# SWivid/F5-TTS

Hardware: NVIDIA H100
Metric: mel_frames_per_sec (higher is better)
Workload: dtype fp16 operands / fp32 accumulate+state

## Files before the change

### f5_tts_b200/csrc/attn.cuh

```cuda
#pragma once
#include "common.cuh"
#include "kparams.h"
#include "wgmma.cuh"

namespace f5 {

__device__ __forceinline__ float ex2_approx(float x) {
  float y;
  asm("ex2.approx.ftz.f32 %0, %1;" : "=f"(y) : "f"(x));
  return y;
}

__global__ void __launch_bounds__(kAttnThreads, 1)
attn_fwd_wgmma_kernel(const __grid_constant__ CUtensorMap tmQKV, const AttnParams p) {
  extern __shared__ uint8_t smem_raw[];
  const uint32_t base = (smem_u32(smem_raw) + 1023u) & ~1023u;
  uint8_t* smem = smem_raw + (base - smem_u32(smem_raw));
  uint8_t* sQ = smem;
  uint8_t* sK = sQ + kAttnTile;
  uint8_t* sV = sK + kAttnStages * kAttnTile;
  uint64_t* bars = reinterpret_cast<uint64_t*>(sV + kAttnStages * kAttnTile);
  uint64_t* q_full = bars;
  uint64_t* k_full = q_full + 1;
  uint64_t* k_empty = k_full + kAttnStages;
  uint64_t* v_full = k_empty + kAttnStages;
  uint64_t* v_empty = v_full + kAttnStages;

  const int warp = threadIdx.x >> 5;
  const int qb = blockIdx.x, h = blockIdx.y, b = blockIdx.z;
  const int q0 = qb * kAttnBQ;
  const int col_q = h * 64, col_k = p.inner + h * 64, col_v = 2 * p.inner + h * 64;

  if (warp == 8 && elect_one()) {
    tma_prefetch_desc(&tmQKV);
    mbar_init(q_full, 1);
    for (int s = 0; s < kAttnStages; ++s) {
      mbar_init(&k_full[s], 1);
      mbar_init(&k_empty[s], 8);
      mbar_init(&v_full[s], 1);
      mbar_init(&v_empty[s], 8);
    }
    fence_mbar_init();
  }
  __syncthreads();
  pdl_wait();
  pdl_launch_dependents();
  const int kv_len = p.kv_len ? max(1, min(p.kv_len[b], p.seq)) : p.seq;
  const int n_kv = (kv_len + kAttnBKV - 1) / kAttnBKV;

  if (warp == 8) {
    if (elect_one()) {
      mbar_expect_tx(q_full, kAttnTile);
      tma_load_3d(sQ, &tmQKV, q_full, col_q, q0, b);
      for (int j = 0; j < n_kv; ++j) {
        const int s = j % kAttnStages;
        const uint32_t ph = (j / kAttnStages) & 1;
        mbar_wait(&k_empty[s], ph ^ 1);
        mbar_expect_tx(&k_full[s], kAttnTile);
        tma_load_3d(sK + s * kAttnTile, &tmQKV, &k_full[s], col_k, j * kAttnBKV, b);
        mbar_wait(&v_empty[s], ph ^ 1);
        mbar_expect_tx(&v_full[s], kAttnTile);
        tma_load_3d(sV + s * kAttnTile, &tmQKV, &v_full[s], col_v, j * kAttnBKV, b);
      }
    }
    return;
  }

  const int g = warp >> 2;
  const int lane = int(lane_id());
  const int r = 64 * g + 16 * (warp & 3) + (lane >> 2);
  const int c2 = 2 * (lane & 3);
  const uint64_t qdesc = make_wgmma_desc_sw128(smem_u32(sQ + g * (64 * 128)));
  float o[32];
#pragma unroll
  for (int i = 0; i < 32; ++i) o[i] = 0.0f;
  float m_run[2] = {-INFINITY, -INFINITY}, l_run[2] = {0.0f, 0.0f};
  mbar_wait(q_full, 0);
  for (int j = 0; j < n_kv; ++j) {
    const int s = j % kAttnStages;
    const uint32_t ph = (j / kAttnStages) & 1;
    const int kv_rem = kv_len - j * kAttnBKV;
    float sc[64];
    mbar_wait(&k_full[s], ph);
    const uint64_t kdesc = make_wgmma_desc_sw128(smem_u32(sK + s * kAttnTile));
    wgmma_fence();
#pragma unroll
    for (int k = 0; k < 4; ++k) wgmma_ss_n128(sc, qdesc + uint64_t(2 * k), kdesc + uint64_t(2 * k), k != 0);
    wgmma_commit();
    wgmma_wait<0>();
    wgmma_fence_regs(sc);
    __syncwarp();
    if (lane == 0) mbar_arrive(&k_empty[s]);
    if (kv_rem < kAttnBKV) {
#pragma unroll
      for (int i = 0; i < 64; ++i)
        if (8 * (i >> 2) + c2 + (i & 1) >= kv_rem) sc[i] = -INFINITY;
    }
    float alpha[2];
#pragma unroll
    for (int hr = 0; hr < 2; ++hr) {
      float mx = -INFINITY;
#pragma unroll
      for (int jj = 0; jj < 16; ++jj) mx = fmaxf(mx, fmaxf(sc[4 * jj + 2 * hr], sc[4 * jj + 2 * hr + 1]));
      mx = fmaxf(mx, __shfl_xor_sync(0xffffffffu, mx, 1));
      mx = fmaxf(mx, __shfl_xor_sync(0xffffffffu, mx, 2));
      const float m_new = fmaxf(m_run[hr], mx * p.scale_log2);
      alpha[hr] = ex2_approx(m_run[hr] - m_new);
      m_run[hr] = m_new;
      float sum = 0.0f;
#pragma unroll
      for (int jj = 0; jj < 16; ++jj) {
        const float e0 = ex2_approx(fmaf(sc[4 * jj + 2 * hr], p.scale_log2, -m_new));
        const float e1 = ex2_approx(fmaf(sc[4 * jj + 2 * hr + 1], p.scale_log2, -m_new));
        sc[4 * jj + 2 * hr] = e0;
        sc[4 * jj + 2 * hr + 1] = e1;
        sum += e0 + e1;
      }
      l_run[hr] = l_run[hr] * alpha[hr] + sum;
    }
#pragma unroll
    for (int jj = 0; jj < 8; ++jj) {
      o[4 * jj + 0] *= alpha[0];
      o[4 * jj + 1] *= alpha[0];
      o[4 * jj + 2] *= alpha[1];
      o[4 * jj + 3] *= alpha[1];
    }
    uint32_t pa[8][4];
#pragma unroll
    for (int kk = 0; kk < 8; ++kk) {
      pa[kk][0] = pack_half2(sc[8 * kk + 0], sc[8 * kk + 1]);
      pa[kk][1] = pack_half2(sc[8 * kk + 2], sc[8 * kk + 3]);
      pa[kk][2] = pack_half2(sc[8 * kk + 4], sc[8 * kk + 5]);
      pa[kk][3] = pack_half2(sc[8 * kk + 6], sc[8 * kk + 7]);
    }
    mbar_wait(&v_full[s], ph);
    wgmma_fence();
#pragma unroll
    for (int kk = 0; kk < 8; ++kk)
      wgmma_rs_n64_bt(o, pa[kk], make_wgmma_desc_sw128(smem_u32(sV + s * kAttnTile + kk * 16 * 128)), 1);
    wgmma_commit();
    wgmma_wait<0>();
    wgmma_fence_regs(o);
    __syncwarp();
    if (lane == 0) mbar_arrive(&v_empty[s]);
  }
#pragma unroll
  for (int hr = 0; hr < 2; ++hr) {
    float l = l_run[hr];
    l += __shfl_xor_sync(0xffffffffu, l, 1);
    l += __shfl_xor_sync(0xffffffffu, l, 2);
    const float inv_l = 1.0f / l;
    const int qrow = q0 + r + 8 * hr;
    if (qrow < p.seq) {
      __half* out = p.out + ((long long)b * p.seq + qrow) * p.inner + h * 64 + c2;
#pragma unroll
      for (int jj = 0; jj < 8; ++jj)
        *reinterpret_cast<uint32_t*>(out + 8 * jj) = pack_half2(o[4 * jj + 2 * hr] * inv_l, o[4 * jj + 2 * hr + 1] * inv_l);
    }
  }
}

}
```

### f5_tts_b200/csrc/common.cuh

```cuda
#pragma once
#include <cuda.h>
#include <cuda_fp16.h>
#include <cuda_runtime.h>
#include <stdint.h>
#include <stdio.h>

#ifndef F5_SPIN_TIMEOUT_CYCLES
#define F5_SPIN_TIMEOUT_CYCLES (4000000000LL)
#endif

namespace f5 {

__device__ __forceinline__ uint32_t smem_u32(const void* p) {
  return static_cast<uint32_t>(__cvta_generic_to_shared(p));
}
__device__ __forceinline__ uint32_t lane_id() { return threadIdx.x & 31; }

__device__ __forceinline__ bool elect_one() {
  uint32_t pred = 0;
  asm volatile(
      "{\n\t.reg .pred P;\n\t.reg .b32 R;\n\telect.sync R|P, 0xffffffff;\n\tselp.b32 %0, 1, 0, P;\n\t}\n"
      : "=r"(pred));
  return pred != 0;
}

__device__ __forceinline__ void mbar_init(uint64_t* bar, uint32_t count) {
  asm volatile("mbarrier.init.shared::cta.b64 [%0], %1;" ::"r"(smem_u32(bar)), "r"(count) : "memory");
}
__device__ __forceinline__ void fence_mbar_init() { asm volatile("fence.mbarrier_init.release.cluster;" ::: "memory"); }
__device__ __forceinline__ void mbar_expect_tx(uint64_t* bar, uint32_t bytes) {
  asm volatile("mbarrier.arrive.expect_tx.shared::cta.b64 _, [%0], %1;" ::"r"(smem_u32(bar)), "r"(bytes) : "memory");
}
__device__ __forceinline__ void mbar_arrive(uint64_t* bar) {
  asm volatile("mbarrier.arrive.shared::cta.b64 _, [%0];" ::"r"(smem_u32(bar)) : "memory");
}
__device__ __forceinline__ bool mbar_try_wait(uint64_t* bar, uint32_t parity) {
  uint32_t ok;
  asm volatile(
      "{\n\t.reg .pred P;\n\tmbarrier.try_wait.parity.shared::cta.b64 P, [%1], %2;\n\tselp.b32 %0, 1, 0, P;\n\t}\n"
      : "=r"(ok)
      : "r"(smem_u32(bar)), "r"(parity)
      : "memory");
  return ok != 0;
}
__device__ __forceinline__ void mbar_wait(uint64_t* bar, uint32_t parity) {
  if (mbar_try_wait(bar, parity)) return;
  long long t0 = clock64();
  while (!mbar_try_wait(bar, parity)) {
    if (clock64() - t0 > F5_SPIN_TIMEOUT_CYCLES) __trap();
  }
}

__device__ __forceinline__ bool mbar_test(uint64_t* bar, uint32_t parity) {
  uint32_t ok;
  asm volatile(
      "{\n\t.reg .pred p;\n\tmbarrier.test_wait.parity.shared::cta.b64 p, [%1], %2;\n\tselp.u32 %0, 1, 0, p;\n\t}"
      : "=r"(ok)
      : "r"(smem_u32(bar)), "r"(parity)
      : "memory");
  return ok != 0;
}

__device__ __forceinline__ void fence_proxy_async_smem() { asm volatile("fence.proxy.async.shared::cta;" ::: "memory"); }
__device__ __forceinline__ void fence_proxy_async_all() { asm volatile("fence.proxy.async;" ::: "memory"); }

__device__ __forceinline__ void tma_prefetch_desc(const CUtensorMap* m) {
  asm volatile("prefetch.tensormap [%0];" ::"l"(reinterpret_cast<uint64_t>(m)) : "memory");
}
__device__ __forceinline__ void tma_load_2d(void* smem_dst, const CUtensorMap* m, uint64_t* bar, int c0, int c1) {
  asm volatile(
      "cp.async.bulk.tensor.2d.shared::cluster.global.mbarrier::complete_tx::bytes [%0], [%1, {%3, %4}], [%2];" ::"r"(
          smem_u32(smem_dst)),
      "l"(reinterpret_cast<uint64_t>(m)), "r"(smem_u32(bar)), "r"(c0), "r"(c1)
      : "memory");
}
__device__ __forceinline__ void tma_load_3d(void* smem_dst, const CUtensorMap* m, uint64_t* bar, int c0, int c1,
                                            int c2) {
  asm volatile(
      "cp.async.bulk.tensor.3d.shared::cluster.global.mbarrier::complete_tx::bytes [%0], [%1, {%3, %4, %5}], [%2];" ::
          "r"(smem_u32(smem_dst)),
      "l"(reinterpret_cast<uint64_t>(m)), "r"(smem_u32(bar)), "r"(c0), "r"(c1), "r"(c2)
      : "memory");
}

__device__ __forceinline__ void tma_store_3d(const CUtensorMap* m, const void* smem_src, int c0, int c1, int c2) {
  asm volatile("cp.async.bulk.tensor.3d.global.shared::cta.bulk_group [%0, {%2, %3, %4}], [%1];" ::"l"(
                   reinterpret_cast<uint64_t>(m)),
               "r"(smem_u32(smem_src)), "r"(c0), "r"(c1), "r"(c2)
               : "memory");
}
__device__ __forceinline__ void tma_reduce_add_3d(const CUtensorMap* m, const void* smem_src, int c0, int c1, int c2) {
  asm volatile("cp.reduce.async.bulk.tensor.3d.global.shared::cta.add.tile.bulk_group [%0, {%2, %3, %4}], [%1];" ::"l"(
                   reinterpret_cast<uint64_t>(m)),
               "r"(smem_u32(smem_src)), "r"(c0), "r"(c1), "r"(c2)
               : "memory");
}
__device__ __forceinline__ void tma_store_commit() { asm volatile("cp.async.bulk.commit_group;" ::: "memory"); }
template <int N>
__device__ __forceinline__ void tma_store_wait_read() {
  asm volatile("cp.async.bulk.wait_group.read %0;" ::"n"(N) : "memory");
}
__device__ __forceinline__ void tma_store_wait_all() { asm volatile("cp.async.bulk.wait_group 0;" ::: "memory"); }
__device__ __forceinline__ void named_bar_sync(int id, int nthreads) {
  asm volatile("bar.sync %0, %1;" ::"r"(id), "r"(nthreads) : "memory");
}

__device__ __forceinline__ void tma_load_2d_multicast(void* smem_dst, const CUtensorMap* m, uint64_t* bar, int c0, int c1,
                                                      uint16_t cta_mask) {
  asm volatile(
      "cp.async.bulk.tensor.2d.shared::cluster.global.mbarrier::complete_tx::bytes.multicast::cluster [%0], [%1, {%3, "
      "%4}], [%2], %5;" ::"r"(smem_u32(smem_dst)),
      "l"(reinterpret_cast<uint64_t>(m)), "r"(smem_u32(bar)), "r"(c0), "r"(c1), "h"(cta_mask)
      : "memory");
}

__device__ __forceinline__ uint32_t cluster_ctarank() {
  uint32_t r;
  asm volatile("mov.u32 %0, %%cluster_ctarank;" : "=r"(r));
  return r;
}
__device__ __forceinline__ void cluster_sync_all() {
  asm volatile("barrier.cluster.arrive.release.aligned;\n\tbarrier.cluster.wait.acquire.aligned;" ::: "memory");
}
__device__ __forceinline__ void mbar_arrive_cluster(uint64_t* bar, uint32_t rank) {
  asm volatile(
      "{\n\t.reg .b32 ra;\n\tmapa.shared::cluster.u32 ra, %0, %1;\n\t"
      "mbarrier.arrive.release.cluster.shared::cluster.b64 _, [ra];\n\t}\n" ::"r"(smem_u32(bar)),
      "r"(rank)
      : "memory");
}

__device__ __forceinline__ void pdl_wait() { asm volatile("griddepcontrol.wait;" ::: "memory"); }
__device__ __forceinline__ void pdl_launch_dependents() { asm volatile("griddepcontrol.launch_dependents;" ::: "memory"); }

__device__ __forceinline__ uint64_t make_wgmma_desc_sw128(uint32_t smem_addr) {
  uint64_t d = 0;
  d |= uint64_t((smem_addr & 0x3FFFF) >> 4);
  d |= uint64_t(1) << 16;
  d |= uint64_t(1024 >> 4) << 32;
  d |= uint64_t(1) << 62;
  return d;
}

__device__ __forceinline__ float gelu_tanh(float x) {
  const float c0 = -2.3022081981f;
  const float c1 = -0.1029432396f;
  float e;
  asm("ex2.approx.ftz.f32 %0, %1;" : "=f"(e) : "f"(x * fmaf(x * x, c1, c0)));
  return __fdividef(x, 1.0f + e);
}
__device__ __forceinline__ float gelu_erf(float x) { return 0.5f * x * (1.0f + erff(x * 0.7071067811865476f)); }
__device__ __forceinline__ float silu(float x) { return x / (1.0f + __expf(-x)); }
__device__ __forceinline__ float mish(float x) {
  float sp = x > 20.0f ? x : log1pf(__expf(x));
  return x * tanhf(sp);
}
__device__ __forceinline__ uint32_t pack_half2(float a, float b) {
  __half2 h = __floats2half2_rn(a, b);
  return *reinterpret_cast<uint32_t*>(&h);
}
__device__ __forceinline__ float warp_sum(float v) {
#pragma unroll
  for (int o = 16; o > 0; o >>= 1) v += __shfl_xor_sync(0xffffffffu, v, o);
  return v;
}
__device__ __forceinline__ float warp_max(float v) {
#pragma unroll
  for (int o = 16; o > 0; o >>= 1) v = fmaxf(v, __shfl_xor_sync(0xffffffffu, v, o));
  return v;
}

}
```

### f5_tts_b200/csrc/kparams.h

```cpp
#pragma once
#include <cuda_fp16.h>
#include <stddef.h>
#include <stdint.h>

namespace f5 {

enum : int { ACT_NONE = 0, ACT_GELU_TANH = 1, ACT_GELU_ERF = 2, ACT_MISH = 3 };
enum : int {
  EPI_F16 = 0,
  EPI_F32 = 1,
  EPI_RESID = 2,
  EPI_QKV_ROPE = 3,
};

struct GemmParams {
  int rows;
  int n_out;
  int num_kb;
  int batches;
  const float* bias;
  void* out;
  __half* out16b;
  float* resid;
  int ldo;
  const float* gate;
  const int* step_ptr;
  long long gate_step_stride;
  const int* row_len;
  int seq;
  const float* rope_cos;
  const float* rope_sin;
  int inner;
  int pe_heads;
  int conv_pad;
  int skip_pad;
  int w_prefetch;
#ifdef F5_TRACE
  int diag_no_epi;
#endif
};

constexpr int kBM = 128;
constexpr int kBK = 64;


struct AttnParams {
  int seq;
  int heads;
  int batches;
  int inner;
  const int* kv_len;
  float scale_log2;
  __half* out;
};

constexpr int kAttnThreads = 288;
constexpr int kAttnBQ = 128;
constexpr int kAttnBKV = 128;
constexpr int kAttnStages = 3;
constexpr uint32_t kAttnTile = 128 * 64 * 2;
constexpr size_t kAttnSmem = size_t(kAttnTile) * (1 + 2 * kAttnStages) + 1024 + 256;

}
```

Baseline: 6972.

## Pipeline attention softmax with next QK GEMM, add warpgroup ping-pong and register split

Restructures the attention consumer loop so the QK^T GEMM for the next KV tile is issued together with the PV GEMM of the current tile. Softmax of the new scores then runs while the PV wgmma is still in flight, in the style of FlashAttention-3 intra-warpgroup pipelining. It also adds named-barrier ping-pong between the two consumer warpgroups so their tensor-core issue alternates. The producer grows to a full warpgroup (384 threads) so setmaxnreg can move registers from the producer to the consumers. The costs are higher register pressure from keeping sc, pa and o live at once, and a more intricate barrier protocol that could deadlock or serialize.

```diff
diff --git a/f5_tts_b200/csrc/attn.cuh b/f5_tts_b200/csrc/attn.cuh
--- a/f5_tts_b200/csrc/attn.cuh
+++ b/f5_tts_b200/csrc/attn.cuh
@@ -9,6 +9,46 @@
   float y;
   asm("ex2.approx.ftz.f32 %0, %1;" : "=f"(y) : "f"(x));
   return y;
+}
+
+__device__ __forceinline__ void attn_softmax_tile(float (&sc)[64], int kv_rem, int c2, float scale_log2,
+                                                  float (&m_run)[2], float (&l_run)[2], float (&alpha)[2]) {
+  if (kv_rem < kAttnBKV) {
+#pragma unroll
+    for (int i = 0; i < 64; ++i)
+      if (8 * (i >> 2) + c2 + (i & 1) >= kv_rem) sc[i] = -INFINITY;
+  }
+#pragma unroll
+  for (int hr = 0; hr < 2; ++hr) {
+    float mx = -INFINITY;
+#pragma unroll
+    for (int jj = 0; jj < 16; ++jj) mx = fmaxf(mx, fmaxf(sc[4 * jj + 2 * hr], sc[4 * jj + 2 * hr + 1]));
+    mx = fmaxf(mx, __shfl_xor_sync(0xffffffffu, mx, 1));
+    mx = fmaxf(mx, __shfl_xor_sync(0xffffffffu, mx, 2));
+    const float m_new = fmaxf(m_run[hr], mx * scale_log2);
+    alpha[hr] = ex2_approx(m_run[hr] - m_new);
+    m_run[hr] = m_new;
+    float sum = 0.0f;
+#pragma unroll
+    for (int jj = 0; jj < 16; ++jj) {
+      const float e0 = ex2_approx(fmaf(sc[4 * jj + 2 * hr], scale_log2, -m_new));
+      const float e1 = ex2_approx(fmaf(sc[4 * jj + 2 * hr + 1], scale_log2, -m_new));
+      sc[4 * jj + 2 * hr] = e0;
+      sc[4 * jj + 2 * hr + 1] = e1;
+      sum += e0 + e1;
+    }
+    l_run[hr] = l_run[hr] * alpha[hr] + sum;
+  }
+}
+
+__device__ __forceinline__ void attn_pack_p(const float (&sc)[64], uint32_t (&pa)[8][4]) {
+#pragma unroll
+  for (int kk = 0; kk < 8; ++kk) {
+    pa[kk][0] = pack_half2(sc[8 * kk + 0], sc[8 * kk + 1]);
+    pa[kk][1] = pack_half2(sc[8 * kk + 2], sc[8 * kk + 3]);
+    pa[kk][2] = pack_half2(sc[8 * kk + 4], sc[8 * kk + 5]);
+    pa[kk][3] = pack_half2(sc[8 * kk + 6], sc[8 * kk + 7]);
+  }
 }
 
 __global__ void __launch_bounds__(kAttnThreads, 1)
@@ -48,8 +88,9 @@
   const int kv_len = p.kv_len ? max(1, min(p.kv_len[b], p.seq)) : p.seq;
   const int n_kv = (kv_len + kAttnBKV - 1) / kAttnBKV;
 
-  if (warp == 8) {
-    if (elect_one()) {
+  if (warp >= 8) {
+    setmaxnreg_dec<kAttnProducerRegs>();
+    if (warp == 8 && elect_one()) {
       mbar_expect_tx(q_full, kAttnTile);
       tma_load_3d(sQ, &tmQKV, q_full, col_q, q0, b);
       for (int j = 0; j < n_kv; ++j) {
@@ -65,59 +106,69 @@
     }
     return;
   }
+  setmaxnreg_inc<kAttnConsumerRegs>();
 
   const int g = warp >> 2;
   const int lane = int(lane_id());
   const int r = 64 * g + 16 * (warp & 3) + (lane >> 2);
   const int c2 = 2 * (lane & 3);
   const uint64_t qdesc = make_wgmma_desc_sw128(smem_u32(sQ + g * (64 * 128)));
+  int turns_left = n_kv + 1;
+  auto mma_turn_begin = [&]() { named_bar_sync(1 + g, 256); };
+  auto mma_turn_end = [&]() {
+    if (--turns_left > 0 || g == 0) named_bar_arrive(2 - g, 256);
+  };
+  if (g == 1) named_bar_arrive(1, 256);
   float o[32];
 #pragma unroll
   for (int i = 0; i < 32; ++i) o[i] = 0.0f;
   float m_run[2] = {-INFINITY, -INFINITY}, l_run[2] = {0.0f, 0.0f};
+  float sc[64];
+  float alpha[2];
+  uint32_t pa[8][4];
+
   mbar_wait(q_full, 0);
-  for (int j = 0; j < n_kv; ++j) {
-    const int s = j % kAttnStages;
-    const uint32_t ph = (j / kAttnStages) & 1;
-    const int kv_rem = kv_len - j * kAttnBKV;
-    float sc[64];
-    mbar_wait(&k_full[s], ph);
-    const uint64_t kdesc = make_wgmma_desc_sw128(smem_u32(sK + s * kAttnTile));
+  mbar_wait(&k_full[0], 0);
+  mma_turn_begin();
+  wgmma_fence();
+#pragma unroll
+  for (int k = 0; k < 4; ++k)
+    wgmma_ss_n128(sc, qdesc + uint64_t(2 * k), make_wgmma_desc_sw128(smem_u32(sK)) + uint64_t(2 * k), k != 0);
+  wgmma_commit();
+  mma_turn_end();
+  wgmma_wait<0>();
+  wgmma_fence_regs(sc);
+  __syncwarp();
+  if (lane == 0) mbar_arrive(&k_empty[0]);
+  attn_softmax_tile(sc, kv_len, c2, p.scale_log2, m_run, l_run, alpha);
+  attn_pack_p(sc, pa);
+
+  for (int j = 0; j + 1 < n_kv; ++j) {
+    const int s = j % kAttnStages, s1 = (j + 1) % kAttnStages;
+    mbar_wait(&k_full[s1], ((j + 1) / kAttnStages) & 1);
+    mbar_wait(&v_full[s], (j / kAttnStages) & 1);
+    const uint64_t kdesc = make_wgmma_desc_sw128(smem_u32(sK + s1 * kAttnTile));
+    const uint64_t vdesc = make_wgmma_desc_sw128(smem_u32(sV + s * kAttnTile));
+    mma_turn_begin();
     wgmma_fence();
 #pragma unroll
     for (int k = 0; k < 4; ++k) wgmma_ss_n128(sc, qdesc + uint64_t(2 * k), kdesc + uint64_t(2 * k), k != 0);
     wgmma_commit();
-    wgmma_wait<0>();
+#pragma unroll
+    for (int kk = 0; kk < 8; ++kk)
+      wgmma_rs_n64_bt(o, pa[kk], vdesc + uint64_t(kk * 128), 1);
+    wgmma_commit();
+    mma_turn_end();
+    wgmma_wait<1>();
     wgmma_fence_regs(sc);
     __syncwarp();
-    if (lane == 0) mbar_arrive(&k_empty[s]);
-    if (kv_rem < kAttnBKV) {
-#pragma unroll
-      for (int i = 0; i < 64; ++i)
-        if (8 * (i >> 2) + c2 + (i & 1) >= kv_rem) sc[i] = -INFINITY;
-    }
-    float alpha[2];
-#pragma unroll
-    for (int hr = 0; hr < 2; ++hr) {
-      float mx = -INFINITY;
-#pragma unroll
-      for (int jj = 0; jj < 16; ++jj) mx = fmaxf(mx, fmaxf(sc[4 * jj + 2 * hr], sc[4 * jj + 2 * hr + 1]));
-      mx = fmaxf(mx, __shfl_xor_sync(0xffffffffu, mx, 1));
-      mx = fmaxf(mx, __shfl_xor_sync(0xffffffffu, mx, 2));
-      const float m_new = fmaxf(m_run[hr], mx * p.scale_log2);
-      alpha[hr] = ex2_approx(m_run[hr] - m_new);
-      m_run[hr] = m_new;
-      float sum = 0.0f;
-#pragma unroll
-      for (int jj = 0; jj < 16; ++jj) {
-        const float e0 = ex2_approx(fmaf(sc[4 * jj + 2 * hr], p.scale_log2, -m_new));
-        const float e1 = ex2_approx(fmaf(sc[4 * jj + 2 * hr + 1], p.scale_log2, -m_new));
-        sc[4 * jj + 2 * hr] = e0;
-        sc[4 * jj + 2 * hr + 1] = e1;
-        sum += e0 + e1;
-      }
-      l_run[hr] = l_run[hr] * alpha[hr] + sum;
-    }
+    if (lane == 0) mbar_arrive(&k_empty[s1]);
+    attn_softmax_tile(sc, kv_len - (j + 1) * kAttnBKV, c2, p.scale_log2, m_run, l_run, alpha);
+    wgmma_wait<0>();
+    wgmma_fence_regs(o);
+    wgmma_fence_regs(sc);
+    __syncwarp();
+    if (lane == 0) mbar_arrive(&v_empty[s]);
 #pragma unroll
     for (int jj = 0; jj < 8; ++jj) {
       o[4 * jj + 0] *= alpha[0];
@@ -125,20 +176,20 @@
       o[4 * jj + 2] *= alpha[1];
       o[4 * jj + 3] *= alpha[1];
     }
-    uint32_t pa[8][4];
-#pragma unroll
-    for (int kk = 0; kk < 8; ++kk) {
-      pa[kk][0] = pack_half2(sc[8 * kk + 0], sc[8 * kk + 1]);
-      pa[kk][1] = pack_half2(sc[8 * kk + 2], sc[8 * kk + 3]);
-      pa[kk][2] = pack_half2(sc[8 * kk + 4], sc[8 * kk + 5]);
-      pa[kk][3] = pack_half2(sc[8 * kk + 6], sc[8 * kk + 7]);
-    }
-    mbar_wait(&v_full[s], ph);
+    attn_pack_p(sc, pa);
+  }
+
+  {
+    const int j = n_kv - 1;
+    const int s = j % kAttnStages;
+    mbar_wait(&v_full[s], (j / kAttnStages) & 1);
+    const uint64_t vdesc = make_wgmma_desc_sw128(smem_u32(sV + s * kAttnTile));
+    mma_turn_begin();
     wgmma_fence();
 #pragma unroll
-    for (int kk = 0; kk < 8; ++kk)
-      wgmma_rs_n64_bt(o, pa[kk], make_wgmma_desc_sw128(smem_u32(sV + s * kAttnTile + kk * 16 * 128)), 1);
+    for (int kk = 0; kk < 8; ++kk) wgmma_rs_n64_bt(o, pa[kk], vdesc + uint64_t(kk * 128), 1);
     wgmma_commit();
+    mma_turn_end();
     wgmma_wait<0>();
     wgmma_fence_regs(o);
     __syncwarp();
diff --git a/f5_tts_b200/csrc/common.cuh b/f5_tts_b200/csrc/common.cuh
--- a/f5_tts_b200/csrc/common.cuh
+++ b/f5_tts_b200/csrc/common.cuh
@@ -104,6 +104,18 @@
 __device__ __forceinline__ void named_bar_sync(int id, int nthreads) {
   asm volatile("bar.sync %0, %1;" ::"r"(id), "r"(nthreads) : "memory");
 }
+__device__ __forceinline__ void named_bar_arrive(int id, int nthreads) {
+  asm volatile("bar.arrive %0, %1;" ::"r"(id), "r"(nthreads) : "memory");
+}
+
+template <uint32_t R>
+__device__ __forceinline__ void setmaxnreg_dec() {
+  asm volatile("setmaxnreg.dec.sync.aligned.u32 %0;" ::"n"(R));
+}
+template <uint32_t R>
+__device__ __forceinline__ void setmaxnreg_inc() {
+  asm volatile("setmaxnreg.inc.sync.aligned.u32 %0;" ::"n"(R));
+}
 
 __device__ __forceinline__ void tma_load_2d_multicast(void* smem_dst, const CUtensorMap* m, uint64_t* bar, int c0, int c1,
                                                       uint16_t cta_mask) {
diff --git a/f5_tts_b200/csrc/kparams.h b/f5_tts_b200/csrc/kparams.h
--- a/f5_tts_b200/csrc/kparams.h
+++ b/f5_tts_b200/csrc/kparams.h
@@ -54,10 +54,13 @@
   __half* out;
 };
 
-constexpr int kAttnThreads = 288;
+constexpr int kAttnThreads = 384;
 constexpr int kAttnBQ = 128;
 constexpr int kAttnBKV = 128;
 constexpr int kAttnStages = 3;
+constexpr int kAttnProducerRegs = 40;
+constexpr int kAttnConsumerRegs = 232;
+static_assert(128 * kAttnProducerRegs + 256 * kAttnConsumerRegs == kAttnThreads * 168, "unbalanced register split");
 constexpr uint32_t kAttnTile = 128 * 64 * 2;
 constexpr size_t kAttnSmem = size_t(kAttnTile) * (1 + 2 * kAttnStages) + 1024 + 256;
 
```

Result: faster. 7089, median of 6 (+1.7%).

## Drop producer warp, issue TMA refills from consumers, fit two CTAs per SM

Applied to the files above, without the earlier changes.

Removes the dedicated TMA producer warp. Thread 0 preloads the first stages, and whichever consumer warp is last to release a stage, counted with a shared-memory atomic, issues that stage's refill. Stages drop from 3 to 2 and launch bounds now ask for 2 CTAs per SM, cutting shared memory and threads per CTA so two attention CTAs can be resident and overlap each other's latency. A partial last Q tile now runs only one consumer warpgroup. The costs are a shallower prefetch pipeline, refill issue sitting on the consumer critical path, and tighter register limits, with atomics and fences replacing mbarriers for the empty signal.

```diff
diff --git a/f5_tts_b200/csrc/attn.cuh b/f5_tts_b200/csrc/attn.cuh
--- a/f5_tts_b200/csrc/attn.cuh
+++ b/f5_tts_b200/csrc/attn.cuh
@@ -11,7 +11,7 @@
   return y;
 }
 
-__global__ void __launch_bounds__(kAttnThreads, 1)
+__global__ void __launch_bounds__(kAttnThreads, 2)
 attn_fwd_wgmma_kernel(const __grid_constant__ CUtensorMap tmQKV, const AttnParams p) {
   extern __shared__ uint8_t smem_raw[];
   const uint32_t base = (smem_u32(smem_raw) + 1023u) & ~1023u;
@@ -22,23 +22,24 @@
   uint64_t* bars = reinterpret_cast<uint64_t*>(sV + kAttnStages * kAttnTile);
   uint64_t* q_full = bars;
   uint64_t* k_full = q_full + 1;
-  uint64_t* k_empty = k_full + kAttnStages;
-  uint64_t* v_full = k_empty + kAttnStages;
-  uint64_t* v_empty = v_full + kAttnStages;
+  uint64_t* v_full = k_full + kAttnStages;
+  uint32_t* k_done = reinterpret_cast<uint32_t*>(v_full + kAttnStages);
+  uint32_t* v_done = k_done + kAttnStages;
 
   const int warp = threadIdx.x >> 5;
   const int qb = blockIdx.x, h = blockIdx.y, b = blockIdx.z;
   const int q0 = qb * kAttnBQ;
   const int col_q = h * 64, col_k = p.inner + h * 64, col_v = 2 * p.inner + h * 64;
 
-  if (warp == 8 && elect_one()) {
+  const int n_act = p.seq - q0 > 64 ? 2 : 1;
+  if (threadIdx.x == 0) {
     tma_prefetch_desc(&tmQKV);
     mbar_init(q_full, 1);
     for (int s = 0; s < kAttnStages; ++s) {
       mbar_init(&k_full[s], 1);
-      mbar_init(&k_empty[s], 8);
       mbar_init(&v_full[s], 1);
-      mbar_init(&v_empty[s], 8);
+      k_done[s] = 0;
+      v_done[s] = 0;
     }
     fence_mbar_init();
   }
@@ -48,26 +49,42 @@
   const int kv_len = p.kv_len ? max(1, min(p.kv_len[b], p.seq)) : p.seq;
   const int n_kv = (kv_len + kAttnBKV - 1) / kAttnBKV;
 
-  if (warp == 8) {
-    if (elect_one()) {
-      mbar_expect_tx(q_full, kAttnTile);
-      tma_load_3d(sQ, &tmQKV, q_full, col_q, q0, b);
-      for (int j = 0; j < n_kv; ++j) {
-        const int s = j % kAttnStages;
-        const uint32_t ph = (j / kAttnStages) & 1;
-        mbar_wait(&k_empty[s], ph ^ 1);
-        mbar_expect_tx(&k_full[s], kAttnTile);
-        tma_load_3d(sK + s * kAttnTile, &tmQKV, &k_full[s], col_k, j * kAttnBKV, b);
-        mbar_wait(&v_empty[s], ph ^ 1);
-        mbar_expect_tx(&v_full[s], kAttnTile);
-        tma_load_3d(sV + s * kAttnTile, &tmQKV, &v_full[s], col_v, j * kAttnBKV, b);
+  const int g = warp >> 2;
+  if (g >= n_act) return;
+  const int lane = int(lane_id());
+  auto load_k = [&](int j) {
+    const int s = j % kAttnStages;
+    mbar_expect_tx(&k_full[s], kAttnTile);
+    tma_load_3d(sK + s * kAttnTile, &tmQKV, &k_full[s], col_k, j * kAttnBKV, b);
+  };
+  auto load_v = [&](int j) {
+    const int s = j % kAttnStages;
+    mbar_expect_tx(&v_full[s], kAttnTile);
+    tma_load_3d(sV + s * kAttnTile, &tmQKV, &v_full[s], col_v, j * kAttnBKV, b);
+  };
+  if (threadIdx.x == 0) {
+    mbar_expect_tx(q_full, kAttnTile);
+    tma_load_3d(sQ, &tmQKV, q_full, col_q, q0, b);
+    for (int j = 0; j < min(n_kv, kAttnStages); ++j) {
+      load_k(j);
+      load_v(j);
+    }
+  }
+  auto release = [&](uint32_t* done, int j, bool is_k) {
+    __syncwarp();
+    if (lane == 0) {
+      __threadfence_block();
+      const uint32_t prev = atomicAdd(&done[j % kAttnStages], 1u);
+      if ((prev + 1) % uint32_t(4 * n_act) == 0 && j + kAttnStages < n_kv) {
+        __threadfence_block();
+        if (is_k)
+          load_k(j + kAttnStages);
+        else
+          load_v(j + kAttnStages);
       }
     }
-    return;
-  }
+  };
 
-  const int g = warp >> 2;
-  const int lane = int(lane_id());
   const int r = 64 * g + 16 * (warp & 3) + (lane >> 2);
   const int c2 = 2 * (lane & 3);
   const uint64_t qdesc = make_wgmma_desc_sw128(smem_u32(sQ + g * (64 * 128)));
@@ -89,8 +106,7 @@
     wgmma_commit();
     wgmma_wait<0>();
     wgmma_fence_regs(sc);
-    __syncwarp();
-    if (lane == 0) mbar_arrive(&k_empty[s]);
+    release(k_done, j, true);
     if (kv_rem < kAttnBKV) {
 #pragma unroll
       for (int i = 0; i < 64; ++i)
@@ -141,8 +157,7 @@
     wgmma_commit();
     wgmma_wait<0>();
     wgmma_fence_regs(o);
-    __syncwarp();
-    if (lane == 0) mbar_arrive(&v_empty[s]);
+    release(v_done, j, false);
   }
 #pragma unroll
   for (int hr = 0; hr < 2; ++hr) {
diff --git a/f5_tts_b200/csrc/kparams.h b/f5_tts_b200/csrc/kparams.h
--- a/f5_tts_b200/csrc/kparams.h
+++ b/f5_tts_b200/csrc/kparams.h
@@ -54,10 +54,10 @@
   __half* out;
 };
 
-constexpr int kAttnThreads = 288;
+constexpr int kAttnThreads = 256;
 constexpr int kAttnBQ = 128;
 constexpr int kAttnBKV = 128;
-constexpr int kAttnStages = 3;
+constexpr int kAttnStages = 2;
 constexpr uint32_t kAttnTile = 128 * 64 * 2;
 constexpr size_t kAttnSmem = size_t(kAttnTile) * (1 + 2 * kAttnStages) + 1024 + 256;
 
```

New measurement: 6910 before, 7098 after (median of 6 runs). +2.7%, better.
